# ADVRHumanoids/CentroidalPlanner

Hardware: AMD Instinct MI355X
Metric: NLP eval_g+eval_jac_g throughput (rows/sec) at batch*contacts; HBM GB/s vs peak (higher is better)
Workload: dtype f64; 1 GPU; 4-contact Ground env, batch=1,048,576 (north-star target); contacts=4, environment=ground, batch_per_gpu=1048576, batch_total=1048576, outputs=g + jac (IFOPT CSR values), per-shard residual norms, parallelism=instance-sharded x1, launch=hip-graph, 10 steps per replay

## Files before the change

centroidalplanner_amd/csrc/cpl_kernels.hip:

```cpp
#include <hip/hip_runtime.h>

#include <cmath>
#include <cstdlib>
#include <cstring>
#include <map>
#include <mutex>
#include <string>
#include <tuple>
#include <vector>

#include "cpl_accept.hpp"
#include "cpl_kkt_block.hpp"
#include "cpl_kkt_wave.hpp"
#include "cpl_layout.hpp"
#include "cpl_wave.hpp"
#include "cpl_status.hpp"

namespace cpl {

constexpr int TILE = 64;
constexpr int CHUNK = 16;
constexpr int SROW = CHUNK + 2;

struct KParams {
// ... 723 lines not shown
        __builtin_nontemporal_store(v.y, &d2[e].y);
      } else {
        d2[e] = s2[e];
      }
    }
    if ((count & 1) && tid == 0) dst[count - 1] = src[count - 1];
  } else {
    for (int e = tid; e < count; e += WG) dst[e] = src[e];
  }
}

template <int WG, bool NT>
__device__ __forceinline__ void copy_out_rows(double* __restrict__ dst, const long long* __restrict__ rowb,
                                              const double* __restrict__ src, int rec, int valid, int tid) {
  const int r2 = rec >> 1;
  const int wave = tid >> 6, lane = tid & 63;
  const double2* s2 = reinterpret_cast<const double2*>(src);
  for (int r = wave; r < valid; r += WG / 64) {
    const int b = __builtin_amdgcn_readfirstlane((int)rowb[r]);
    double2* d = reinterpret_cast<double2*>(dst + (int64_t)b * rec);
    const double2* sr = s2 + r * r2;
    for (int q = lane; q < r2; q += 64) {
      const double2 v = sr[q];
      if (NT) {
        __builtin_nontemporal_store(v.x, &d[q].x);
        __builtin_nontemporal_store(v.y, &d[q].y);
      } else {
        d[q] = v;
      }
    }
  }
}

template <int ENVK>
__device__ __forceinline__ void contact_item(const KParams& K, const double* __restrict__ xr, int kind, int k,
                                             double* __restrict__ Gr, double* __restrict__ Jr) {
  const int i = s_ct.map_order[k];
  const double* q = xr + 3 + 9 * i;
  const double F0 = q[0], F1 = q[1], F2 = q[2];
  const double p0 = q[3], p1 = q[4], p2 = q[5];
  const double n0 = q[6], n1 = q[7], n2 = q[8];
  const bool wg = K.want_g, wj = K.want_j;
  double* gk = Gr + 6 + (K.has_env ? 6 : 2) * k;
  double* jk = Jr + K.jbase + K.cstride * k;
  if (ENVK != CPL_ENV_NONE) {
    double gv[4], ej[3], nj[3][3];
    if (ENVK == CPL_ENV_GROUND || (ENVK == CPL_ENV_MIXED && kind == CPL_ENV_GROUND)) {
      gv[0] = p2 - K.ground_z;
      gv[1] = n0 - 0.0; gv[2] = n1 - 0.0; gv[3] = n2 - 1.0;
      ej[0] = 0.0; ej[1] = 0.0; ej[2] = 1.0;
#pragma unroll
      for (int r = 0; r < 3; ++r)
#pragma unroll
        for (int c = 0; c < 3; ++c) nj[r][c] = 0.0;
    } else {
      SQContact s;
      superquadric_contact(K, p0, p1, p2, wj, s);
      gv[0] = s.val;
      gv[1] = n0 - s.en[0]; gv[2] = n1 - s.en[1]; gv[3] = n2 - s.en[2];
#pragma unroll
      for (int r = 0; r < 3; ++r) {
        ej[r] = s.ej[r];
#pragma unroll
        for (int c = 0; c < 3; ++c) nj[r][c] = wj ? s.nj[r][c] : 0.0;
      }
    }
    if (wg) { gk[0] = gv[0]; gk[1] = gv[1]; gk[2] = gv[2]; gk[3] = gv[3]; }
    if (wj && K.fold == FOLD_NONE) {
      jk[0] = ej[0]; jk[1] = ej[1]; jk[2] = ej[2];
#pragma unroll
      for (int r = 0; r < 3; ++r) {
        jk[3 + 4 * r] = nj[r][0]; jk[4 + 4 * r] = nj[r][1]; jk[5 + 4 * r] = nj[r][2]; jk[6 + 4 * r] = 1.0;
      }
      jk += 15;
    } else if (wj && K.fold == FOLD_COMMON) {
      jk[0] = ej[0]; jk[1] = ej[1]; jk[2] = ej[2];
#pragma unroll
      for (int r = 0; r < 3; ++r) { jk[3 + 3 * r] = nj[r][0]; jk[4 + 3 * r] = nj[r][1]; jk[5 + 3 * r] = nj[r][2]; }
      jk += 12;
    }
    gk += 4;
  }
  const double mu = K.mu;
  const double t1 = dot3(F0, F1, F2, n0, n1, n2);
  if (wg) {
    const double nF = dot3(n0, n1, n2, F0, F1, F2);
    const double u0 = F0 - nF * n0, u1 = F1 - nF * n1, u2 = F2 - nF * n2;
    gk[0] = -t1 + s_ct.F_thr[i];
    gk[1] = sqrt((u0 * u0 + u1 * u1) + u2 * u2) - mu * t1;
  }
  if (wj) {
    const double t2 = F0 - n0 * t1;
    const double t3 = F1 - n1 * t1;
    const double t4 = F2 - n2 * t1;
    const double t5 = F0 * n0;
    const double t6 = F1 * n1;
    const double t7 = F2 * n2;
    const double s = sqrt(t2 * t2 + t3 * t3 + t4 * t4);
    jk[0] = -n0; jk[1] = -n1; jk[2] = -n2;
    jk[3] = -F0; jk[4] = -F1; jk[5] = -F2;
    jk[6] = (t2 * (n0 * n0 - 1.0) * 2.0 + n0 * n1 * t3 * 2.0 + n0 * n2 * t4 * 2.0) * 1.0 / s * (-1.0 / 2.0) - mu * n0;
    jk[7] = (t3 * (n1 * n1 - 1.0) * 2.0 + n0 * n1 * t2 * 2.0 + n1 * n2 * t4 * 2.0) * 1.0 / s * (-1.0 / 2.0) - mu * n1;
    jk[8] = (t4 * (n2 * n2 - 1.0) * 2.0 + n0 * n2 * t2 * 2.0 + n1 * n2 * t3 * 2.0) * 1.0 / s * (-1.0 / 2.0) - mu * n2;
    jk[9] = (t2 * (t6 + t7 + t5 * 2.0) * 2.0 + F0 * n1 * t3 * 2.0 + F0 * n2 * t4 * 2.0) * 1.0 / s * (-1.0 / 2.0) - mu * F0;
    jk[10] = (t3 * (t5 + t7 + t6 * 2.0) * 2.0 + F1 * n0 * t2 * 2.0 + F1 * n2 * t4 * 2.0) * 1.0 / s * (-1.0 / 2.0) - mu * F1;
    jk[11] = (t4 * (t5 + t6 + t7 * 2.0) * 2.0 + F2 * n0 * t2 * 2.0 + F2 * n1 * t3 * 2.0) * 1.0 / s * (-1.0 / 2.0) - mu * F2;
  }
}

struct TemplateSrc {
  __device__ __forceinline__ double wrench(const KParams& K, int t) const { return K.wrench[t]; }
  __device__ __forceinline__ double com_ref(const KParams& K, int a) const { return K.com_ref[a]; }
  __device__ __forceinline__ double p_ref(const KParams& K, int i, int a) const { return K.p_ref[i][a]; }
  __device__ __forceinline__ double F_ref(const KParams& K, int i, int a) const { return K.F_ref[i][a]; }
};
struct InstSrc {
  const double* w;
  const double* c;
  const double* p;
  const double* F;
  __device__ __forceinline__ double wrench(const KParams&, int t) const { return w[t]; }
  __device__ __forceinline__ double com_ref(const KParams&, int a) const { return c[a]; }
  __device__ __forceinline__ double p_ref(const KParams&, int i, int a) const { return p[3 * i + a]; }
  __device__ __forceinline__ double F_ref(const KParams&, int i, int a) const { return F[3 * i + a]; }
};

template <class SRC = TemplateSrc>
__device__ __forceinline__ void statics_values_item(const KParams& K, const double* __restrict__ xr, double m_i,
                                                    double* __restrict__ Gr, double* __restrict__ Jr,
                                                    bool with_j = true, double* __restrict__ com6 = nullptr,
                                                    bool pairs_j = false, const SRC& src = SRC()) {
  const int N = K.N;
  if (pairs_j && K.want_j) {
    com6 = Jr + (K.fold == FOLD_NONE ? 3 * N : 0);
  }
  const bool pairs = com6 != nullptr, vals = K.want_g != 0;
  if (pairs || vals) {
    const double c0 = xr[0], c1 = xr[1], c2 = xr[2];
    double v0 = 0.0, v1 = 0.0, v2 = 0.0, v3 = 0.0, v4 = 0.0, v5 = 0.0;
    double a[6] = {0.0, 0.0, 0.0, 0.0, 0.0, 0.0};
    for (int k0 = 0; k0 < N; k0 += 4) {
      double q[4][6];
#pragma unroll
      for (int u = 0; u < 4; ++u) {
        const double* qq = xr + 3 + 9 * s_ct.map_order[k0 + u < N ? k0 + u : k0];
#pragma unroll
        for (int e = 0; e < 6; ++e) q[u][e] = qq[e];
      }
#pragma unroll
      for (int u = 0; u < 4; ++u) {
        if (k0 + u >= N) break;
        const double F0 = q[u][0], F1 = q[u][1], F2 = q[u][2];
        if (pairs) {
          a[0] -= -(-1.0) * F2; a[1] -= -(1.0) * F1;
          a[2] -= -(1.0) * F2;  a[3] -= -(-1.0) * F0;
          a[4] -= -(-1.0) * F1; a[5] -= -(1.0) * F0;
        }
        if (vals) {
          const double d0 = q[u][3] - c0, d1 = q[u][4] - c1, d2 = q[u][5] - c2;
          v0 += F0; v1 += F1; v2 += F2;
          v3 += d1 * F2 - d2 * F1;
          v4 += d2 * F0 - d0 * F2;
          v5 += d0 * F1 - d1 * F0;
        }
      }
    }
    if (pairs) {
      if (pairs_j) {
#pragma unroll
        for (int t = 0; t < 6; ++t) com6[(t >> 1) * (2 + 4 * N) + (t & 1)] = a[t];
      } else {
#pragma unroll
        for (int t = 0; t < 6; ++t) com6[t] = a[t];
      }
    }
    if (vals) {
      v0 -= src.wrench(K, 0); v1 -= src.wrench(K, 1); v2 -= src.wrench(K, 2);
      v3 -= src.wrench(K, 3); v4 -= src.wrench(K, 4); v5 -= src.wrench(K, 5);
      v0 += m_i * K.gravity[0]; v1 += m_i * K.gravity[1]; v2 += m_i * K.gravity[2];
      Gr[0] = v0; Gr[1] = v1; Gr[2] = v2; Gr[3] = v3; Gr[4] = v4; Gr[5] = v5;
    }
  }
  if (with_j && K.want_j && K.fold == FOLD_NONE)
    for (int e = 0; e < 3 * N; ++e) Jr[e] = 1.0;
}

__device__ __forceinline__ void statics_rows_coop(const KParams& K, const double* __restrict__ xr,
                                                  const double* __restrict__ com6, double* __restrict__ Jr, int tid,
                                                  int nthreads) {
  const int N = K.N;
  const int RL = 2 + 4 * N;
  const int I3 = K.fold == FOLD_NONE ? 3 * N : 0;
  const int SJ = I3 + 3 * RL;
  for (int e = tid; e < SJ; e += nthreads) {
    double v = 1.0;
    if (e >= I3) {
      int w = e - I3;
      const int q = w >= 2 * RL ? 2 : (w >= RL ? 1 : 0);
      w -= q * RL;
      const int e1 = q == 2 ? 1 : 2;
      const int e2 = q == 0 ? 1 : 0;
      const double s1 = q == 1 ? 1.0 : -1.0;
      const double s2 = q == 1 ? -1.0 : 1.0;
      if (w < 2) {
        v = com6[2 * q + w];
      } else {
        const int i = (w - 2) >> 2, c = (w - 2) & 3;
        const double* F = xr + 3 + 9 * i;
        const double* p = F + 3;
        v = c == 0 ? s1 * (p[e1] - xr[e1]) : c == 1 ? s2 * (p[e2] - xr[e2]) : c == 2 ? -s1 * F[e1] : -s2 * F[e2];
      }
    }
    Jr[e] = v;
  }
}

__device__ __forceinline__ void statics_row_item(const KParams& K, const double* __restrict__ xr, int q,
                                                 double* __restrict__ Jr) {
  const int N = K.N;
  const int e1 = q == 2 ? 1 : 2;
  const int e2 = q == 0 ? 1 : 0;
  const double s1 = q == 1 ? 1.0 : -1.0;
  const double s2 = q == 1 ? -1.0 : 1.0;
  const double ce1 = xr[e1], ce2 = xr[e2];
  double a1 = 0.0, a2 = 0.0;
  for (int k = 0; k < N; ++k) {
    const double* F = xr + 3 + 9 * s_ct.map_order[k];
    a1 -= -s1 * F[e1];
    a2 -= -s2 * F[e2];
  }
  double* row = Jr + (K.fold == FOLD_NONE ? 3 * N : 0) + q * (2 + 4 * N);
  row[0] = a1;
  row[1] = a2;
  for (int i = 0; i < N; ++i) {
    const double* F = xr + 3 + 9 * i;
    const double* p = F + 3;
    row[2 + 4 * i] = s1 * (p[e1] - ce1);
    row[3 + 4 * i] = s2 * (p[e2] - ce2);
    row[4 + 4 * i] = -s1 * F[e1];
    row[5 + 4 * i] = -s2 * F[e2];
  }
}

template <class SRC = TemplateSrc>
__device__ __forceinline__ double cost_value(const KParams& K, const double* __restrict__ xr, const SRC& src = SRC()) {
  const int N = K.N;
  double value = 0;
  for (int k = 0; k < N; ++k) {
    const int i = s_ct.map_order[k];
    const double* q = xr + 3 + 9 * i;
    const double e0 = q[3] - src.p_ref(K, i, 0), e1 = q[4] - src.p_ref(K, i, 1), e2 = q[5] - src.p_ref(K, i, 2);
    const double h0 = q[0] - src.F_ref(K, i, 0), h1 = q[1] - src.F_ref(K, i, 1), h2 = q[2] - src.F_ref(K, i, 2);
    value += 0.5 * K.W_p[i] * ((e0 * e0 + e1 * e1) + e2 * e2) + 0.5 * K.W_F[i] * ((h0 * h0 + h1 * h1) + h2 * h2);
  }
  const double r0 = xr[0] - src.com_ref(K, 0), r1 = xr[1] - src.com_ref(K, 1), r2 = xr[2] - src.com_ref(K, 2);
  value += 0.5 * K.W_com * ((r0 * r0 + r1 * r1) + r2 * r2);
  return value;
}

template <class SRC = TemplateSrc>
__device__ __forceinline__ void cost_item(const KParams& K, const double* __restrict__ xr, double* __restrict__ f,
                                          double* __restrict__ Dr, const double* __restrict__ fscale = nullptr,
                                          const SRC& src = SRC()) {
  const int N = K.N;
// ... 626 lines not shown
    }
    if (K.want_lgrad) {
      for (int e = tid; e < valid * n; e += CT) {
        const int r = e / n, j = e - r * n;
        if (K.lg_active && !K.lg_active[(b0 + r) / K.y_repeat]) continue;
        const double* jr = Jt + r * nnz;
        const double* yb = K.ly + ((b0 + r) / K.y_repeat) * m;
        double s = Dt[r * n + j];
        for (int q = s_colp[j]; q < s_colp[j + 1]; ++q) {
          double v = jr[s_csck[q]];
          v = v == v ? v : 0.0;
          s += v * yb[s_cscr[q]];
        }
        grad_out[(b0 + r) * n + j] = s;
      }
    } else if (K.soa) {
      if (K.want_g) copy_out_soa<CT, NT>(g_out + b0, batch, Gt, m, valid, tid);
      if (K.want_j) copy_out_soa<CT, NT>(jac_out + b0, batch, Jt, nnz, valid, tid);
      if (K.want_grad) copy_out_soa<CT, NT>(grad_out + b0, batch, Dt, n, valid, tid);
    } else {
      if (K.want_g) copy_out_ct<CT, NT>(g_out + b0 * m, Gt, valid * m, tid);
      if (K.want_j) copy_out_ct<CT, NT>(jac_out + b0 * nnz, Jt, valid * nnz, tid);
      if (K.want_grad) copy_out_ct<CT, NT>(grad_out + b0 * n, Dt, valid * n, tid);
    }
    if (K.want_norms) acc.add_tile(Gt, valid * m, tid, CT, m);
    lds_barrier();
    cur ^= 1;
  }
  }
  if (K.want_norms) partial_norms(acc, norms_ws + NORM_HDR);
}
using PipeKernT = void (*)(const KParams, int64_t, const double*, const double*, const uint8_t*, double*, double*,
                           double*, double*, double*);


constexpr int ENT_PC = 15;
enum { EPC_D = 0, EPC_ROW1 = 3, EPC_CONEG = 9, EPC_ENVG = 11, EPC_NORMG = 12 };
constexpr unsigned OP_X = 0u << 28, OP_S = 1u << 28, OP_C = 2u << 28, OP_NEG = 1u << 31;

template <int ENVK>
__device__ __forceinline__ unsigned entry_op_g(int q, int S0) {
  constexpr int CR = ENVK == CPL_ENV_NONE ? 2 : 6;
  if (q < 6) return OP_S | (unsigned)q;
  const int u = q - 6, k = u / CR, w = u - k * CR;
  const unsigned ci = (unsigned)(S0 + ENT_PC * s_ct.map_order[k]);
  if (ENVK == CPL_ENV_NONE) return OP_S | (ci + EPC_CONEG + w);
  if (w == 0) return OP_S | (ci + EPC_ENVG);
  if (w < 4) return OP_S | (ci + EPC_NORMG + (w - 1));
  return OP_S | (ci + EPC_CONEG + (w - 4));
}
template <int ENVK>
__device__ __forceinline__ unsigned entry_op_j(int q, int N, int S0) {
  constexpr int CJ = ENVK == CPL_ENV_NONE ? 12 : 27;
  const int RL = 2 + 4 * N, JC = 3 * N + 3 * RL;
  if (q < 3 * N) return OP_C | 1u;
  if (q < JC) {
    int w = q - 3 * N;
    const int qq = w >= 2 * RL ? 2 : (w >= RL ? 1 : 0);
    w -= qq * RL;
    if (w < 2) return OP_S | (unsigned)(6 + 2 * qq + w);
    const int e1 = qq == 2 ? 1 : 2, e2 = qq == 0 ? 1 : 0;
    const bool s1neg = qq != 1, s2neg = qq == 1;
    const int i = (w - 2) >> 2, c = (w - 2) & 3;
    const unsigned ci = (unsigned)(S0 + ENT_PC * i);
    switch (c) {
      case 0: return OP_S | (ci + EPC_D + e1) | (s1neg ? OP_NEG : 0u);
// ... 737 lines not shown
    K.C[a] = C; K.R[a] = R; K.P[a] = P;
    if (sq) {
      K.EJ[a] = cache.EJ[a]; K.Ka[a] = cache.Ka[a]; K.Kb[a] = cache.Kb[a];
      K.Rm2[a] = cache.Rm2[a]; K.Rp2[a] = cache.Rp2[a];
    }
    K.Psq[a] = P * P;
    K.Pm1[a] = P - 1.0;
    K.P2[a] = P * 2.0;
    K.P2m2[a] = P * 2.0 - 2.0;
    K.P2m3[a] = P * 2.0 - 3.0;
  }
  K.sq_ladder = 1;
  for (int a = 0; a < 3; ++a) {
    const double P = d->sq_P[a];
    if (!(P >= 2.0 && P <= 64.0 && P == std::floor(P))) K.sq_ladder = 0;
  }
  for (int i = 0; i < CPL_MAX_CONTACTS; ++i) {
    K.F_thr[i] = d->F_thr[i];
    K.W_p[i] = d->W_p[i];
    K.W_F[i] = d->W_F[i];
    for (int j = 0; j < 3; ++j) { K.p_ref[i][j] = d->p_ref[i][j]; K.F_ref[i][j] = d->F_ref[i][j]; }
  }
  K.W_com = d->W_com;
  for (int j = 0; j < 3; ++j) K.com_ref[j] = d->com_ref[j];
  K.fold = FOLD_NONE;
  K.jbase = D.statics_nnz;
  K.cstride = D.contact_nnz;
  K.soa = 0;
}

static size_t eval_lds_bytes(int n) { return sizeof(double) * (size_t)(TILE * n + 2 * TILE * SROW); }

enum { VAR_AUTO = 0, VAR_ROWSTAGE = 1, VAR_PIPE = 2, VAR_TILE = 3, VAR_TILE_JD = 4, VAR_ENTRY = 5, VAR_SPLIT = 6,
       VAR_SPLIT_JD = 7 };
static int g_variant = VAR_AUTO;
static size_t g_lds_budget = 0;
static int g_wg = 256;
static int g_nt = 1;

static size_t tile_budget() { return g_lds_budget ? g_lds_budget : 48 * 1024; }
static size_t pipe_budget() { return g_lds_budget ? g_lds_budget : 48 * 1024; }
static bool use_rowstage() { return g_variant == VAR_ROWSTAGE; }
static bool use_pipe(const KParams& K) {
  if (!K.x_aligned16) return false;
  if (g_variant == VAR_PIPE) return true;
  return g_variant == VAR_AUTO && (K.env_kind == CPL_ENV_NONE || K.env_kind == CPL_ENV_GROUND);
}

static int32_t plan_tile(KParams& K, bool g, bool j, bool f, bool grad, int t_max = 64, bool size_without_j = false) {
  const size_t budget = tile_budget();
  K.want_g = g; K.want_j = j; K.want_f = f; K.want_grad = grad;
  const bool sq = K.env_kind == CPL_ENV_SUPERQUADRIC || K.env_kind == CPL_ENV_MIXED;
  K.LR = K.N * SQ_L + 1;
  const size_t per = sizeof(double) * (size_t)(K.n + (g ? K.m : 0) + (j && !K.jdirect ? K.nnz : 0) +
                                               (grad ? K.n : 0) + (sq ? K.LR : 0) + (j && K.jdirect ? 6 : 0));
  const size_t per_t = size_without_j ? per - sizeof(double) * (size_t)(j && !K.jdirect ? K.nnz : 0) : per;
  const size_t fixed = sizeof(double) * 72 + sizeof(CTab);
  int T = 64, logT = 6;
  while (T > t_max) { T >>= 1; --logT; }
  while (T > 2 && (size_t)T * per_t + fixed > budget) { T >>= 1; --logT; }
  if ((size_t)T * per + fixed > 160 * 1024) return fail(CPL_ERR_UNSUPPORTED, "problem too large for one LDS tile");
  K.T = T; K.logT = logT;
  K.cost_seg = (f || grad) ? K.N + 4 : -1;
  K.S = K.N + 4 + ((f || grad) ? 1 : 0);
  K.offG = T * K.n;
  K.offJ = K.offG + (g ? T * K.m : 0);
  K.offD = K.offJ + (j && !K.jdirect ? T * K.nnz : 0);
  K.offL = K.offD + (grad ? T * K.n : 0);
  K.offA = K.offL + (sq ? T * K.LR : 0);
  K.offI = K.offA + (j && K.jdirect ? 6 * T : 0);
  K.offI = (K.offI + 1) & ~1;
  K.offRB = K.offI + 72;
  return CPL_OK;
}

static int32_t plan_pipe(KParams& K, bool g, bool j, bool f, bool grad, size_t extra_fixed = 0) {
  K.want_g = g; K.want_j = j; K.want_f = f; K.want_grad = grad;
  const bool sq = K.env_kind == CPL_ENV_SUPERQUADRIC || K.env_kind == CPL_ENV_MIXED;
// ... 140 lines not shown
  if (c.norms && (st = norm_workspace(C, c.stream, nparts, &ws))) return st;
  if ((st = side_stream(C, c.stream))) return st;
  hipError_t e = hipEventRecord(C.fork, c.stream);
  if (e == hipSuccess) e = hipStreamWaitEvent(C.side, C.fork, 0);
  if (e != hipSuccess) return hip_fail(e, "mixed split fork");
  hipLaunchKernelGGL(tk, dim3(grid_s), dim3(256), lds_s, c.stream, Ks, batch, c.x, c.mass, c.env_tag, kl.idx_sq,
                     kl.counts + 1, c.g, c.jac, c.f, c.grad, ws ? ws + 2 * (size_t)grid_g : nullptr);
  hipLaunchKernelGGL(ek, dim3(grid_g), dim3(256), lds_g, C.side, Kg, batch, c.x, c.mass, kl.idx_gr, kl.counts, c.g,
                     c.jac, c.f, c.grad, ws);
  e = hipGetLastError();
  if (e != hipSuccess) return hip_fail(e, "mixed split launch");
  e = hipEventRecord(C.join, C.side);
  if (e == hipSuccess) e = hipStreamWaitEvent(c.stream, C.join, 0);
  if (e != hipSuccess) return hip_fail(e, "mixed split join");
  return launched(c, "mixed split launch", nparts, ws);
}

static int32_t launch_entry(const EvalCall& c, KParams& K, StreamCtx* C) {
  int32_t st = plan_entry(K, c.g != nullptr, c.jac != nullptr, c.f != nullptr, c.grad != nullptr);
  if (st) return st;
  const size_t lds = sizeof(double) * (size_t)K.offI;
  static const EntryKernT table[2][2] = {
      {cpl_eval_entry_kernel<CPL_ENV_NONE, false>, cpl_eval_entry_kernel<CPL_ENV_NONE, true>},
      {cpl_eval_entry_kernel<CPL_ENV_GROUND, false>, cpl_eval_entry_kernel<CPL_ENV_GROUND, true>}};
  const EntryKernT kern = table[K.env_kind == CPL_ENV_GROUND ? 1 : 0][g_nt ? 1 : 0];
  const unsigned grid = persistent_grid((c.batch + K.T - 1) / K.T, reinterpret_cast<const void*>(kern), lds);
  double* ws = nullptr;
  if (c.norms && (st = norm_workspace(*C, c.stream, grid, &ws))) return st;
  hipLaunchKernelGGL(kern, dim3(grid), dim3(256), lds, c.stream, K, c.batch, c.x, c.mass, nullptr, nullptr, c.g, c.jac,
                     c.f, c.grad, ws);
  return launched(c, "cpl_eval_entry_kernel launch", grid, ws);
}

static int32_t launch_pipe(const EvalCall& c, KParams& K, StreamCtx* C) {
  const LGradArgs* lg = c.lg;
  const int csc_doubles = lg ? (K.n + 1 + 2 * K.nnz + 1) / 2 : 0;
  int32_t st = lg ? plan_pipe(K, false, true, false, true, sizeof(double) * (size_t)csc_doubles)
                  : plan_pipe(K, c.g != nullptr, c.jac != nullptr, c.f != nullptr, c.grad != nullptr);
  if (st) return st;
  K.offC = K.offI + 72;
  if (lg) {
    K.want_lgrad = 1;
    K.y_repeat = lg->y_repeat;
    K.col_ptr = lg->col_ptr;
    K.csc_k = lg->csc_k;
    K.csc_row = lg->csc_row;
    K.ly = lg->y;
    K.lg_active = lg->active;
  }
  const size_t lds = sizeof(double) * (size_t)(K.offC + csc_doubles);
  static const PipeKernT table[4][2] = {
      {cpl_eval_pipe_kernel<CPL_ENV_NONE, 3, false>, cpl_eval_pipe_kernel<CPL_ENV_NONE, 3, true>},
      {cpl_eval_pipe_kernel<CPL_ENV_GROUND, 3, false>, cpl_eval_pipe_kernel<CPL_ENV_GROUND, 3, true>},
      {cpl_eval_pipe_kernel<CPL_ENV_SUPERQUADRIC, 3, false>, cpl_eval_pipe_kernel<CPL_ENV_SUPERQUADRIC, 3, true>},
      {cpl_eval_pipe_kernel<CPL_ENV_MIXED, 3, false>, cpl_eval_pipe_kernel<CPL_ENV_MIXED, 3, true>}};
  static const PipeKernT table_sc[2][2] = {
      {cpl_eval_pipe_kernel<CPL_ENV_NONE, 3, false, true>, cpl_eval_pipe_kernel<CPL_ENV_NONE, 3, true, true>},
      {cpl_eval_pipe_kernel<CPL_ENV_GROUND, 3, false, true>, cpl_eval_pipe_kernel<CPL_ENV_GROUND, 3, true, true>}};
  if (c.sc && K.env_kind != CPL_ENV_NONE && K.env_kind != CPL_ENV_GROUND) return CPL_ERR_UNSUPPORTED;
  if (c.sc) {
    K.sc_df = c.sc->df;
    K.sc_dc = c.sc->dc;
    K.sc_row = c.sc->row;
  }
  const PipeKernT kern =
      c.sc ? table_sc[K.env_kind == CPL_ENV_GROUND ? 1 : 0][g_nt ? 1 : 0] : table[K.env_kind][g_nt ? 1 : 0];
  const unsigned grid = persistent_grid((c.batch + K.T - 1) / K.T, reinterpret_cast<const void*>(kern), lds);
  double* ws = nullptr;
  if (c.norms && (st = norm_workspace(*C, c.stream, grid, &ws))) return st;
  hipLaunchKernelGGL(kern, dim3(grid), dim3(256), lds, c.stream, K, c.batch, c.x, c.mass, c.env_tag, c.g, c.jac, c.f,
                     c.grad, ws);
  return launched(c, "cpl_eval_pipe_kernel launch", grid, ws);
}

static int32_t launch_rowstage(const EvalCall& c, const KParams& K) {
  const size_t lds = eval_lds_bytes(K.n);
  if (lds > 160 * 1024) return fail(CPL_ERR_UNSUPPORTED, "problem too large for one LDS tile");
  const unsigned grid = (unsigned)((c.batch + TILE - 1) / TILE);
  hipLaunchKernelGGL(cpl_eval_kernel, dim3(grid), dim3(TILE), lds, c.stream, K, c.batch, c.x, c.mass, c.env_tag, c.g,
                     c.jac, c.f, c.grad);
  if (int32_t st = launched(c, "cpl_eval_kernel launch")) return st;
  return c.norms && c.finish ? cpl_residual_norms(c.d, c.batch, c.g, c.norms, c.stream) : CPL_OK;
}

static int32_t launch_tile(const EvalCall& c, KParams& K, StreamCtx* C) {
  const bool jd = g_variant == VAR_TILE_JD || (g_variant == VAR_AUTO && K.env_kind == CPL_ENV_MIXED);
  const int wg = g_wg;
  K.jdirect = (jd && c.jac && !K.soa && wg == 256) ? 1 : 0;
  int32_t st = plan_tile(K, c.g != nullptr, c.jac != nullptr, c.f != nullptr, c.grad != nullptr, 64, jd && c.jac);
  if (st) return st;
  const size_t lds = sizeof(double) * (size_t)(K.offRB + K.T);
  const unsigned grid = (unsigned)((c.batch + K.T - 1) / K.T);
  const size_t nparts = (size_t)grid * (wg / 64);
  double* ws = nullptr;
  if (c.norms && (st = norm_workspace(*C, c.stream, nparts, &ws))) return st;
#define CPL_TILE_KERNELS(E) \
  {cpl_eval_tile_kernel<E, 128, false, false>, cpl_eval_tile_kernel<E, 128, true, false>,        \
   cpl_eval_tile_kernel<E, 256, false, false>, cpl_eval_tile_kernel<E, 256, true, false>,        \
   cpl_eval_tile_kernel<E, 256, false, true>, cpl_eval_tile_kernel<E, 256, true, true>}
// ... 11 lines not shown
  int32_t st = validate_desc(d);
  if (st) return st;
  if (c.flags & ~(CPL_EVAL_JAC_FOLDED | CPL_EVAL_SOA)) return fail(CPL_ERR_INVALID_ARGUMENT, "unknown eval flags");
  if (c.batch < 0) return fail(CPL_ERR_INVALID_ARGUMENT, "negative batch");
  if (c.batch == 0) {
    if (c.norms) {
      hipError_t e = hipMemsetAsync(c.norms, 0, 2 * sizeof(double), c.stream);
      if (e != hipSuccess) return hip_fail(e, "hipMemsetAsync norms");
    }
    return CPL_OK;
  }
  if (c.norms && !c.g) return fail(CPL_ERR_INVALID_ARGUMENT, "residual norms need the g output");
  if (!c.x) return fail(CPL_ERR_INVALID_ARGUMENT, "x is required");
  if (d->env_kind == CPL_ENV_MIXED && !c.env_tag)
    return fail(CPL_ERR_INVALID_ARGUMENT, "mixed environment batch needs a per-instance env tag array");
  if ((c.batch + 7) / 8 > 0x7fffffffLL) return fail(CPL_ERR_INVALID_ARGUMENT, "batch too large");
  if (!c.g && !c.jac && !c.f && !c.grad) return CPL_OK;
  KParams K;
  fill_params(d, K, c.x);
  K.gate = c.gate;
  if (c.flags & CPL_EVAL_JAC_FOLDED) {
    K.fold = fold_level(d->env_kind);
    K.nnz = folded_nnz(K.N, d->env_kind);
    K.jbase = 6 + 12 * K.N;
    K.cstride = folded_contact_nnz(d->env_kind);
  }
  K.soa = (c.flags & CPL_EVAL_SOA) ? 1 : 0;
  K.want_norms = c.norms != nullptr;
  K.y_repeat = 1;
  const bool split = !c.lg && use_split(K, c.flags, c.batch), entry = !c.lg && use_entry(K, c.flags);
  if (c.sc && (c.lg || c.norms || K.soa || !use_pipe(K) || split || entry)) return CPL_ERR_UNSUPPORTED;
  if (c.lg && !use_pipe(K))
    return fail(CPL_ERR_UNSUPPORTED, "fused Lagrangian gradient: pipelined (Ground / no environment) path only");
  StreamCtx* C = nullptr;
  if ((split || c.norms) && (st = stream_ctx(c.stream, &C))) return st;
  if (split && (g_variant != VAR_AUTO || split_ready(*C, c.stream, c.batch))) return launch_split(c, K, *C);
  if (entry) return launch_entry(c, K, C);
  if (use_pipe(K)) return launch_pipe(c, K, C);
  if (use_rowstage() && c.flags == 0) return launch_rowstage(c, K);
  return launch_tile(c, K, C);
}

struct InstPtrs {
  const double *wrench, *com_ref, *p_ref, *F_ref;
  bool any() const { return wrench || com_ref || p_ref || F_ref; }
};

template <bool NT>
__global__ __launch_bounds__(256) void cpl_inst_overlay_kernel(const KParams K, int64_t batch,
                                                               const double* __restrict__ x,
                                                               const double* __restrict__ mass, const InstPtrs I,
                                                               double* __restrict__ g_out, double* __restrict__ f_out,
                                                               double* __restrict__ grad_out) {
  extern __shared__ __align__(16) double smem[];
  if (K.gate && *K.gate == 0) return;
  const int tid = threadIdx.x;
  const int T = K.T, n = K.n, m = K.m, N = K.N;
  const int64_t b0 = (int64_t)blockIdx.x * T;
  if (b0 >= batch) return;
  const int valid = (int)((batch - b0) < T ? (batch - b0) : T);
  double* X = smem;
  double* Dt = X + T * n;
  double* G6 = Dt + T * n;
  double* Fv = G6 + T * 6;
  double* Wl = Fv + T;
  double* Cl = Wl + T * 6;
// ... 479 lines not shown
                               void* stream) {
  int32_t st = validate_desc(d);
  if (st) return st;
  if (d->env_kind != CPL_ENV_GROUND && d->env_kind != CPL_ENV_NONE)
    return fail(CPL_ERR_UNSUPPORTED, "cpl_lagrangian_hessian: Ground / no-environment problems only");
  return launch_hessian("cpl_lagrangian_hessian", d, batch, d_x, d_y, nullptr, d_active, d_free_idx, nf, d_H, stream);
}

int32_t cpl_lagrangian_hessian_ex(const cpl_problem_desc* d, int64_t batch, const double* d_x, const double* d_y,
                                  const uint8_t* d_env_tag, const uint8_t* d_active, const int32_t* d_free_idx,
                                  int32_t nf, double* d_H, void* stream) {
  int32_t st = validate_desc(d);
  if (st) return st;
  return launch_hessian("cpl_lagrangian_hessian_ex", d, batch, d_x, d_y, d_env_tag, d_active, d_free_idx, nf, d_H,
                        stream);
}

int32_t cpl_eval_batch_ex(const cpl_problem_desc* d, int64_t batch, const double* d_x, const double* d_mass,
                          const uint8_t* d_env_tag, double* d_g, double* d_jac, double* d_f, double* d_grad,
                          double* d_norms, int32_t flags, void* stream) {
  return launch_eval(EvalCall{d, batch, d_x, d_mass, d_env_tag, d_g, d_jac, d_f, d_grad, d_norms, (hipStream_t)stream, flags});
}

int32_t cpl_eval_batch_norms(const cpl_problem_desc* d, int64_t batch, const double* d_x, const double* d_mass,
                             const uint8_t* d_env_tag, double* d_g, double* d_jac, double* d_f, double* d_grad,
                             double* d_norms, void* stream) {
  if (!d_norms) return fail(CPL_ERR_INVALID_ARGUMENT, "d_norms is required");
  return launch_eval(EvalCall{d, batch, d_x, d_mass, d_env_tag, d_g, d_jac, d_f, d_grad, d_norms, (hipStream_t)stream});
}

int32_t cpl_set_tuning(int32_t kernel_variant, int32_t tile_lds_kb, int32_t wg_threads, int32_t nt_stores,
                       int32_t reserved ) {
  if (reserved != 0) return fail(CPL_ERR_INVALID_ARGUMENT, "the fifth tuning argument is reserved and must be 0");
  if (kernel_variant < VAR_AUTO || kernel_variant > VAR_SPLIT_JD) return fail(CPL_ERR_INVALID_ARGUMENT, "unknown kernel variant");
  if (tile_lds_kb != 0 && (tile_lds_kb < 8 || tile_lds_kb > 160))
    return fail(CPL_ERR_INVALID_ARGUMENT, "LDS budget out of [8, 160] KiB");
  if (wg_threads != 128 && wg_threads != 256) return fail(CPL_ERR_INVALID_ARGUMENT, "workgroup size must be 128 or 256");
  g_variant = kernel_variant;
  g_lds_budget = (size_t)tile_lds_kb * 1024;
  g_wg = wg_threads;
  g_nt = nt_stores ? 1 : 0;
  return CPL_OK;
}

int32_t cpl_residual_norms(const cpl_problem_desc* d, int64_t batch, const double* d_g, double* d_out, void* stream) {
  int32_t st = validate_desc(d);
  if (st) return st;
  if (batch < 0 || !d_out || (batch > 0 && !d_g)) return fail(CPL_ERR_INVALID_ARGUMENT, "bad residual arguments");
  hipStream_t s = (hipStream_t)stream;
  StreamCtx* C = nullptr;
  if ((st = stream_ctx(s, &C))) return st;
  if ((st = ctx_reserve(s, C->rn, RN_GRID, sizeof(double) * 2 * RN_GRID, "residual norms: the per-stream workspace")))
    return st;
  double* ws = static_cast<double*>(C->rn.ptr);
  const Dims D = dims_of(d->n_contacts, d->env_kind);
  const int64_t total = batch * D.m;
  int64_t blocks = (total + RN_BLOCK - 1) / RN_BLOCK;
  if (blocks < 1) blocks = 1;
  if (blocks > RN_GRID) blocks = RN_GRID;
  hipLaunchKernelGGL(cpl_residual_partial, dim3((unsigned)blocks), dim3(RN_BLOCK), 0, s, total, D.m, D.contact_rows,
                     d_g, ws);
  hipError_t e = hipGetLastError();
  if (e != hipSuccess) return hip_fail(e, "cpl_residual_partial launch");
  launch_residual_final((int)blocks, ws, d_out, s);
  e = hipGetLastError();
  if (e != hipSuccess) return hip_fail(e, "cpl_residual_final launch");
  return CPL_OK;
// ... 42 lines not shown
```

Baseline: 78.70 billion rows/s.

## Add fixed-shape pipelined kernel specialised for 4 contacts with hoisted constant Jacobian entries

Adds a compile-time specialised pipelined kernel for N=4 contacts (no environment or Ground). It writes the constant Jacobian entries (ones and ground zeros) into shared memory once per block instead of every tile, and splits the cone Jacobian work across waves. It also uses register-staged copy-out with compile-time trip counts. The default auto path picks this kernel when the layout matches the generic pipe kernel's offsets, at the cost of more code paths and a risk of layout mismatch.

```diff
diff --git a/centroidalplanner_amd/csrc/cpl_kernels.hip b/centroidalplanner_amd/csrc/cpl_kernels.hip
--- a/centroidalplanner_amd/csrc/cpl_kernels.hip
+++ b/centroidalplanner_amd/csrc/cpl_kernels.hip
@@ -779,6 +779,53 @@
   }
 }
 
+struct ConeArgs { double F0, F1, F2, n0, n1, n2; };
+struct ConeTerms { double t2, t3, t4, t5, t6, t7, s; };
+
+__device__ __forceinline__ void ground_values(double p2, double n0, double n1, double n2, double ground_z,
+                                              double* __restrict__ gv) {
+  gv[0] = p2 - ground_z;
+  gv[1] = n0 - 0.0; gv[2] = n1 - 0.0; gv[3] = n2 - 1.0;
+}
+
+__device__ __forceinline__ void cone_values(const ConeArgs& a, double t1, double F_thr, double mu,
+                                            double* __restrict__ gk) {
+  const double F0 = a.F0, F1 = a.F1, F2 = a.F2, n0 = a.n0, n1 = a.n1, n2 = a.n2;
+  const double nF = dot3(n0, n1, n2, F0, F1, F2);
+  const double u0 = F0 - nF * n0, u1 = F1 - nF * n1, u2 = F2 - nF * n2;
+  gk[0] = -t1 + F_thr;
+  gk[1] = sqrt((u0 * u0 + u1 * u1) + u2 * u2) - mu * t1;
+}
+
+__device__ __forceinline__ ConeTerms cone_terms(const ConeArgs& a, double t1) {
+  ConeTerms t;
+  t.t2 = a.F0 - a.n0 * t1;
+  t.t3 = a.F1 - a.n1 * t1;
+  t.t4 = a.F2 - a.n2 * t1;
+  t.t5 = a.F0 * a.n0;
+  t.t6 = a.F1 * a.n1;
+  t.t7 = a.F2 * a.n2;
+  t.s = sqrt(t.t2 * t.t2 + t.t3 * t.t3 + t.t4 * t.t4);
+  return t;
+}
+__device__ __forceinline__ void cone_row0(const ConeArgs& a, double* __restrict__ jk) {
+  jk[0] = -a.n0; jk[1] = -a.n1; jk[2] = -a.n2;
+  jk[3] = -a.F0; jk[4] = -a.F1; jk[5] = -a.F2;
+}
+template <int E>
+__device__ __forceinline__ double cone_row1(const ConeArgs& a, const ConeTerms& t, double mu) {
+  const double F0 = a.F0, F1 = a.F1, F2 = a.F2, n0 = a.n0, n1 = a.n1, n2 = a.n2;
+  const double t2 = t.t2, t3 = t.t3, t4 = t.t4, t5 = t.t5, t6 = t.t6, t7 = t.t7, s = t.s;
+  switch (E) {
+    case 0: return (t2 * (n0 * n0 - 1.0) * 2.0 + n0 * n1 * t3 * 2.0 + n0 * n2 * t4 * 2.0) * 1.0 / s * (-1.0 / 2.0) - mu * n0;
+    case 1: return (t3 * (n1 * n1 - 1.0) * 2.0 + n0 * n1 * t2 * 2.0 + n1 * n2 * t4 * 2.0) * 1.0 / s * (-1.0 / 2.0) - mu * n1;
+    case 2: return (t4 * (n2 * n2 - 1.0) * 2.0 + n0 * n2 * t2 * 2.0 + n1 * n2 * t3 * 2.0) * 1.0 / s * (-1.0 / 2.0) - mu * n2;
+    case 3: return (t2 * (t6 + t7 + t5 * 2.0) * 2.0 + F0 * n1 * t3 * 2.0 + F0 * n2 * t4 * 2.0) * 1.0 / s * (-1.0 / 2.0) - mu * F0;
+    case 4: return (t3 * (t5 + t7 + t6 * 2.0) * 2.0 + F1 * n0 * t2 * 2.0 + F1 * n2 * t4 * 2.0) * 1.0 / s * (-1.0 / 2.0) - mu * F1;
+    default: return (t4 * (t5 + t6 + t7 * 2.0) * 2.0 + F2 * n0 * t2 * 2.0 + F2 * n1 * t3 * 2.0) * 1.0 / s * (-1.0 / 2.0) - mu * F2;
+  }
+}
+
 template <int ENVK>
 __device__ __forceinline__ void contact_item(const KParams& K, const double* __restrict__ xr, int kind, int k,
                                              double* __restrict__ Gr, double* __restrict__ Jr) {
@@ -793,8 +840,7 @@
   if (ENVK != CPL_ENV_NONE) {
     double gv[4], ej[3], nj[3][3];
     if (ENVK == CPL_ENV_GROUND || (ENVK == CPL_ENV_MIXED && kind == CPL_ENV_GROUND)) {
-      gv[0] = p2 - K.ground_z;
-      gv[1] = n0 - 0.0; gv[2] = n1 - 0.0; gv[3] = n2 - 1.0;
+      ground_values(p2, n0, n1, n2, K.ground_z, gv);
       ej[0] = 0.0; ej[1] = 0.0; ej[2] = 1.0;
 #pragma unroll
       for (int r = 0; r < 3; ++r)
@@ -829,31 +875,39 @@
     gk += 4;
   }
   const double mu = K.mu;
+  const ConeArgs a{F0, F1, F2, n0, n1, n2};
   const double t1 = dot3(F0, F1, F2, n0, n1, n2);
-  if (wg) {
-    const double nF = dot3(n0, n1, n2, F0, F1, F2);
-    const double u0 = F0 - nF * n0, u1 = F1 - nF * n1, u2 = F2 - nF * n2;
-    gk[0] = -t1 + s_ct.F_thr[i];
-    gk[1] = sqrt((u0 * u0 + u1 * u1) + u2 * u2) - mu * t1;
-  }
+  if (wg) cone_values(a, t1, s_ct.F_thr[i], mu, gk);
   if (wj) {
-    const double t2 = F0 - n0 * t1;
-    const double t3 = F1 - n1 * t1;
-    const double t4 = F2 - n2 * t1;
-    const double t5 = F0 * n0;
-    const double t6 = F1 * n1;
-    const double t7 = F2 * n2;
-    const double s = sqrt(t2 * t2 + t3 * t3 + t4 * t4);
-    jk[0] = -n0; jk[1] = -n1; jk[2] = -n2;
-    jk[3] = -F0; jk[4] = -F1; jk[5] = -F2;
-    jk[6] = (t2 * (n0 * n0 - 1.0) * 2.0 + n0 * n1 * t3 * 2.0 + n0 * n2 * t4 * 2.0) * 1.0 / s * (-1.0 / 2.0) - mu * n0;
-    jk[7] = (t3 * (n1 * n1 - 1.0) * 2.0 + n0 * n1 * t2 * 2.0 + n1 * n2 * t4 * 2.0) * 1.0 / s * (-1.0 / 2.0) - mu * n1;
-    jk[8] = (t4 * (n2 * n2 - 1.0) * 2.0 + n0 * n2 * t2 * 2.0 + n1 * n2 * t3 * 2.0) * 1.0 / s * (-1.0 / 2.0) - mu * n2;
-    jk[9] = (t2 * (t6 + t7 + t5 * 2.0) * 2.0 + F0 * n1 * t3 * 2.0 + F0 * n2 * t4 * 2.0) * 1.0 / s * (-1.0 / 2.0) - mu * F0;
-    jk[10] = (t3 * (t5 + t7 + t6 * 2.0) * 2.0 + F1 * n0 * t2 * 2.0 + F1 * n2 * t4 * 2.0) * 1.0 / s * (-1.0 / 2.0) - mu * F1;
-    jk[11] = (t4 * (t5 + t6 + t7 * 2.0) * 2.0 + F2 * n0 * t2 * 2.0 + F2 * n1 * t3 * 2.0) * 1.0 / s * (-1.0 / 2.0) - mu * F2;
-  }
-}
+    const ConeTerms t = cone_terms(a, t1);
+    cone_row0(a, jk);
+    jk[6] = cone_row1<0>(a, t, mu);
+    jk[7] = cone_row1<1>(a, t, mu);
+    jk[8] = cone_row1<2>(a, t, mu);
+    jk[9] = cone_row1<3>(a, t, mu);
+    jk[10] = cone_row1<4>(a, t, mu);
+    jk[11] = cone_row1<5>(a, t, mu);
+  }
+}
+
+struct LaunchShape {
+  static constexpr bool writes_constants = true;
+  __device__ __forceinline__ int N(const KParams& K) const { return K.N; }
+  __device__ __forceinline__ bool want_g(const KParams& K) const { return K.want_g != 0; }
+  __device__ __forceinline__ bool want_j(const KParams& K) const { return K.want_j != 0; }
+  __device__ __forceinline__ int fold(const KParams& K) const { return K.fold; }
+  __device__ __forceinline__ int order(int k) const { return s_ct.map_order[k]; }
+};
+template <int NF>
+struct FixedShape {
+  static constexpr bool writes_constants = false;
+  int mo[NF];
+  __device__ __forceinline__ constexpr int N(const KParams&) const { return NF; }
+  __device__ __forceinline__ constexpr bool want_g(const KParams&) const { return true; }
+  __device__ __forceinline__ constexpr bool want_j(const KParams&) const { return true; }
+  __device__ __forceinline__ constexpr int fold(const KParams&) const { return FOLD_NONE; }
+  __device__ __forceinline__ int order(int k) const { return mo[k]; }
+};
 
 struct TemplateSrc {
   __device__ __forceinline__ double wrench(const KParams& K, int t) const { return K.wrench[t]; }
@@ -872,16 +926,17 @@
   __device__ __forceinline__ double F_ref(const KParams&, int i, int a) const { return F[3 * i + a]; }
 };
 
-template <class SRC = TemplateSrc>
+template <class SRC = TemplateSrc, class SH = LaunchShape>
 __device__ __forceinline__ void statics_values_item(const KParams& K, const double* __restrict__ xr, double m_i,
                                                     double* __restrict__ Gr, double* __restrict__ Jr,
                                                     bool with_j = true, double* __restrict__ com6 = nullptr,
-                                                    bool pairs_j = false, const SRC& src = SRC()) {
-  const int N = K.N;
-  if (pairs_j && K.want_j) {
-    com6 = Jr + (K.fold == FOLD_NONE ? 3 * N : 0);
-  }
-  const bool pairs = com6 != nullptr, vals = K.want_g != 0;
+                                                    bool pairs_j = false, const SRC& src = SRC(),
+                                                    const SH& sh = SH()) {
+  const int N = sh.N(K);
+  if (pairs_j && sh.want_j(K)) {
+    com6 = Jr + (sh.fold(K) == FOLD_NONE ? 3 * N : 0);
+  }
+  const bool pairs = com6 != nullptr, vals = sh.want_g(K);
   if (pairs || vals) {
     const double c0 = xr[0], c1 = xr[1], c2 = xr[2];
     double v0 = 0.0, v1 = 0.0, v2 = 0.0, v3 = 0.0, v4 = 0.0, v5 = 0.0;
@@ -890,7 +945,7 @@
       double q[4][6];
 #pragma unroll
       for (int u = 0; u < 4; ++u) {
-        const double* qq = xr + 3 + 9 * s_ct.map_order[k0 + u < N ? k0 + u : k0];
+        const double* qq = xr + 3 + 9 * sh.order(k0 + u < N ? k0 + u : k0);
 #pragma unroll
         for (int e = 0; e < 6; ++e) q[u][e] = qq[e];
       }
@@ -928,7 +983,7 @@
       Gr[0] = v0; Gr[1] = v1; Gr[2] = v2; Gr[3] = v3; Gr[4] = v4; Gr[5] = v5;
     }
   }
-  if (with_j && K.want_j && K.fold == FOLD_NONE)
+  if (SH::writes_constants && with_j && sh.want_j(K) && sh.fold(K) == FOLD_NONE)
     for (int e = 0; e < 3 * N; ++e) Jr[e] = 1.0;
 }
 
@@ -962,9 +1017,10 @@
   }
 }
 
+template <class SH = LaunchShape>
 __device__ __forceinline__ void statics_row_item(const KParams& K, const double* __restrict__ xr, int q,
-                                                 double* __restrict__ Jr) {
-  const int N = K.N;
+                                                 double* __restrict__ Jr, const SH& sh = SH()) {
+  const int N = sh.N(K);
   const int e1 = q == 2 ? 1 : 2;
   const int e2 = q == 0 ? 1 : 0;
   const double s1 = q == 1 ? 1.0 : -1.0;
@@ -972,11 +1028,11 @@
   const double ce1 = xr[e1], ce2 = xr[e2];
   double a1 = 0.0, a2 = 0.0;
   for (int k = 0; k < N; ++k) {
-    const double* F = xr + 3 + 9 * s_ct.map_order[k];
+    const double* F = xr + 3 + 9 * sh.order(k);
     a1 -= -s1 * F[e1];
     a2 -= -s2 * F[e2];
   }
-  double* row = Jr + (K.fold == FOLD_NONE ? 3 * N : 0) + q * (2 + 4 * N);
+  double* row = Jr + (sh.fold(K) == FOLD_NONE ? 3 * N : 0) + q * (2 + 4 * N);
   row[0] = a1;
   row[1] = a2;
   for (int i = 0; i < N; ++i) {
@@ -1669,6 +1725,217 @@
 }
 using PipeKernT = void (*)(const KParams, int64_t, const double*, const double*, const uint8_t*, double*, double*,
                            double*, double*, double*);
+
+template <int ENVK, int N>
+struct PipeFixed {
+  static_assert(ENVK == CPL_ENV_NONE || ENVK == CPL_ENV_GROUND, "fixed-shape kernel: no environment or Ground");
+  static constexpr bool ENV = ENVK != CPL_ENV_NONE;
+  static constexpr int NCW = 3, CT = 64 * NCW;
+  static constexpr int n = 3 + 9 * N, CR = ENV ? 6 : 2, CJ = ENV ? 27 : 12;
+  static constexpr int m = 6 + CR * N, SJ = 6 + 15 * N, nnz = SJ + CJ * N;
+  static constexpr int up2(int v) { return (v + 1) & ~1; }
+  static constexpr int tile_log() {
+    int T = 64, logT = 6;
+    while (T > 8 && sizeof(double) * (size_t)T * (2 * n + 3 + m + nnz) + sizeof(double) * 80 + sizeof(CTab) > 48 * 1024) {
+      T >>= 1;
+      --logT;
+    }
+    return logT;
+  }
+  static constexpr int LOGT = tile_log(), T = 1 << LOGT;
+  static constexpr int offX1 = up2(T * n), offMB = offX1 + up2(T * n), offTB = offMB + 2 * T, offG = offTB + T,
+                       offJ = offG + T * m, offI = up2(offJ + T * nnz);
+  static_assert(m % 2 == 0 && nnz % 2 == 0, "records of whole 16-byte pairs");
+};
+
+template <int CT, bool NT, bool FULL, int PG, int PJ>
+__device__ __forceinline__ void copy_out_fixed(double* __restrict__ g_dst, double* __restrict__ j_dst,
+                                               const double* __restrict__ Gt, const double* __restrict__ Jt, int pg,
+                                               int pj, int tid) {
+  constexpr int TG = (PG + CT - 1) / CT, TJ = (PJ + CT - 1) / CT;
+  const double2* sg = reinterpret_cast<const double2*>(Gt);
+  const double2* sj = reinterpret_cast<const double2*>(Jt);
+  double2* dg = reinterpret_cast<double2*>(g_dst);
+  double2* dj = reinterpret_cast<double2*>(j_dst);
+  double2 vg[TG], vj[TJ];
+#pragma unroll
+  for (int i = 0; i < TG; ++i) vg[i] = sg[(i + 1) * CT <= PG || tid + i * CT < PG ? tid + i * CT : tid];
+#pragma unroll
+  for (int i = 0; i < TJ; ++i) vj[i] = sj[(i + 1) * CT <= PJ || tid + i * CT < PJ ? tid + i * CT : tid];
+  auto put = [](double2* d, const double2 v) {
+    if (NT) {
+      __builtin_nontemporal_store(v.x, &d->x);
+      __builtin_nontemporal_store(v.y, &d->y);
+    } else {
+      *d = v;
+    }
+  };
+#pragma unroll
+  for (int i = 0; i < TG; ++i) {
+    const int e = tid + i * CT;
+    if (FULL ? ((i + 1) * CT <= PG || e < PG) : e < pg) put(dg + e, vg[i]);
+  }
+#pragma unroll
+  for (int i = 0; i < TJ; ++i) {
+    const int e = tid + i * CT;
+    if (FULL ? ((i + 1) * CT <= PJ || e < PJ) : e < pj) put(dj + e, vj[i]);
+  }
+}
+
+template <int ENVK, int N, bool NT>
+__global__ __launch_bounds__(256) void cpl_eval_pipe_fixed_kernel(const KParams K, int64_t batch,
+                                                                  const double* __restrict__ x,
+                                                                  const double* __restrict__ mass,
+                                                                  const uint8_t* __restrict__ ,
+                                                                  double* __restrict__ g_out,
+                                                                  double* __restrict__ jac_out,
+                                                                  double* __restrict__ ,
+                                                                  double* __restrict__ ,
+                                                                  double* __restrict__ norms_ws) {
+  using FS = PipeFixed<ENVK, N>;
+  constexpr int NCW = FS::NCW, CT = FS::CT, T = FS::T, LOGT = FS::LOGT, n = FS::n, m = FS::m, nnz = FS::nnz;
+  constexpr int SJ = FS::SJ, CJ = FS::CJ, CR = FS::CR;
+  constexpr bool ENV = FS::ENV;
+  constexpr int CTRIPS = (N * T + 63) / 64, STRIPS = (4 * T + 63) / 64;
+  extern __shared__ __align__(16) double smem[];
+  load_ctab(K);
+  __syncthreads();
+  const int tid = threadIdx.x;
+  const int lane = tid & 63, wave = tid >> 6;
+  const bool loader = wave == NCW;
+  const int64_t ntiles = (batch + T - 1) >> LOGT;
+  auto XB = [&](int bi) { return smem + (bi ? FS::offX1 : 0); };
+  auto MB = [&](int bi) { return smem + FS::offMB + (bi ? T : 0); };
+  double* Gt = smem + FS::offG;
+  double* Jt = smem + FS::offJ;
+
+  int64_t t = blockIdx.x;
+  if (t >= ntiles) return;
+  double mass_def = K.mass_default;
+  asm volatile("" : "+v"(mass_def));
+  NormAcc acc;
+  acc.init(tid, CT, m);
+
+  if (loader) {
+    double st_mass = 0.0, st_tail = 0.0;
+    auto stage = [&](int64_t tt, int bi) {
+      const int64_t b0s = tt << LOGT;
+      const int vs = (int)((batch - b0s) < T ? (batch - b0s) : T);
+      const int count = vs * n;
+      dma_tile(XB(bi), x + b0s * n, count, lane);
+      if ((count & 1) && lane == 0) st_tail = x[b0s * n + count - 1];
+      if (lane < vs) st_mass = mass ? mass[b0s + lane] : mass_def;
+    };
+    auto finish_stage = [&](int64_t tt, int bi) {
+      asm volatile("s_waitcnt vmcnt(0)" ::: "memory");
+      const int64_t b0s = tt << LOGT;
+      const int vs = (int)((batch - b0s) < T ? (batch - b0s) : T);
+      const int count = vs * n;
+      if ((count & 1) && lane == 0) XB(bi)[count - 1] = st_tail;
+      if (lane < vs) MB(bi)[lane] = st_mass;
+    };
+    __builtin_amdgcn_s_setprio(3);
+    stage(t, 0);
+    finish_stage(t, 0);
+    lds_barrier();
+    int cur = 0;
+    for (; t < ntiles; t += gridDim.x) {
+      const int64_t tn = t + gridDim.x;
+      if (tn < ntiles) stage(tn, cur ^ 1);
+      lds_barrier();
+      if (tn < ntiles) finish_stage(tn, cur ^ 1);
+      lds_barrier();
+      cur ^= 1;
+    }
+  } else {
+    FixedShape<N> sh;
+#pragma unroll
+    for (int k = 0; k < N; ++k) sh.mo[k] = __builtin_amdgcn_readfirstlane(s_ct.map_order[k]);
+    int ci[CTRIPS];
+    double fthr[CTRIPS];
+#pragma unroll
+    for (int u = 0; u < CTRIPS; ++u) {
+      const int k = (lane + 64 * u) >> LOGT;
+      ci[u] = s_ct.map_order[k < N ? k : 0];
+      fthr[u] = s_ct.F_thr[ci[u]];
+    }
+    const double mu = K.mu, ground_z = K.ground_z;
+    for (int e = tid; e < T * 3 * N; e += CT) Jt[(e / (3 * N)) * nnz + e % (3 * N)] = 1.0;
+    if (ENV)
+      for (int e = tid; e < T * N * 15; e += CT) {
+        const int r = e / (N * 15), w = e % (N * 15), c = w % 15;
+        Jt[r * nnz + SJ + CJ * (w / 15) + c] = (c == 2 || (c >= 3 && ((c - 3) & 3) == 3)) ? 1.0 : 0.0;
+      }
+    lds_barrier();
+    int cur = 0;
+    for (; t < ntiles; t += gridDim.x) {
+      const int64_t b0 = t << LOGT;
+      const int valid = (int)((batch - b0) < T ? (batch - b0) : T);
+      const double* X = XB(cur);
+      if (wave < 2) {
+#pragma unroll
+        for (int u = 0; u < CTRIPS; ++u) {
+          const int it = lane + 64 * u, r = it & (T - 1), k = it >> LOGT;
+          if (it >= N * T || r >= valid) continue;
+          const double* q = X + r * n + 3 + 9 * ci[u];
+          const ConeArgs a{q[0], q[1], q[2], q[6], q[7], q[8]};
+          const ConeTerms ct = cone_terms(a, dot3(a.F0, a.F1, a.F2, a.n0, a.n1, a.n2));
+          double* jk = Jt + r * nnz + SJ + CJ * k + (ENV ? 15 : 0);
+          if (wave == 0) {
+            jk[6] = cone_row1<0>(a, ct, mu);
+            jk[7] = cone_row1<1>(a, ct, mu);
+            jk[8] = cone_row1<2>(a, ct, mu);
+          } else {
+            jk[9] = cone_row1<3>(a, ct, mu);
+            jk[10] = cone_row1<4>(a, ct, mu);
+            jk[11] = cone_row1<5>(a, ct, mu);
+          }
+        }
+      } else {
+#pragma unroll
+        for (int u = 0; u < CTRIPS; ++u) {
+          const int it = lane + 64 * u, r = it & (T - 1), k = it >> LOGT;
+          if (it >= N * T || r >= valid) continue;
+          const double* q = X + r * n + 3 + 9 * ci[u];
+          const ConeArgs a{q[0], q[1], q[2], q[6], q[7], q[8]};
+          double* gk = Gt + r * m + 6 + CR * k;
+          double* jk = Jt + r * nnz + SJ + CJ * k;
+          if (ENV) {
+            double gv[4];
+            ground_values(q[5], a.n0, a.n1, a.n2, ground_z, gv);
+            gk[0] = gv[0]; gk[1] = gv[1]; gk[2] = gv[2]; gk[3] = gv[3];
+            gk += 4;
+            jk += 15;
+          }
+          cone_values(a, dot3(a.F0, a.F1, a.F2, a.n0, a.n1, a.n2), fthr[u], mu, gk);
+          cone_row0(a, jk);
+        }
+#pragma unroll
+        for (int u = 0; u < STRIPS; ++u) {
+          const int it = lane + 64 * u, r = it & (T - 1), sg = it >> LOGT;
+          if (it >= 4 * T || r >= valid) continue;
+          const double* xr = X + r * n;
+          if (sg == 0)
+            statics_values_item<TemplateSrc, FixedShape<N>>(K, xr, MB(cur)[r], Gt + r * m, Jt + r * nnz, true, nullptr,
+                                                            false, TemplateSrc(), sh);
+          else
+            statics_row_item(K, xr, sg - 1, Jt + r * nnz, sh);
+        }
+      }
+      lds_barrier();
+      if (valid == T)
+        copy_out_fixed<CT, NT, true, T * m / 2, T * nnz / 2>(g_out + b0 * m, jac_out + b0 * nnz, Gt, Jt, T * m / 2,
+                                                            T * nnz / 2, tid);
+      else
+        copy_out_fixed<CT, NT, false, T * m / 2, T * nnz / 2>(g_out + b0 * m, jac_out + b0 * nnz, Gt, Jt,
+                                                             valid * m / 2, (valid * nnz) >> 1, tid);
+      if (K.want_norms) acc.add_tile(Gt, valid * m, tid, CT, m);
+      lds_barrier();
+      cur ^= 1;
+    }
+  }
+  if (K.want_norms) partial_norms(acc, norms_ws + NORM_HDR);
+}
 
 
 constexpr int ENT_PC = 15;
@@ -2472,7 +2739,7 @@
 static size_t eval_lds_bytes(int n) { return sizeof(double) * (size_t)(TILE * n + 2 * TILE * SROW); }
 
 enum { VAR_AUTO = 0, VAR_ROWSTAGE = 1, VAR_PIPE = 2, VAR_TILE = 3, VAR_TILE_JD = 4, VAR_ENTRY = 5, VAR_SPLIT = 6,
-       VAR_SPLIT_JD = 7 };
+       VAR_SPLIT_JD = 7, VAR_UNASSIGNED = 8 , VAR_PIPE_FIXED = 9 };
 static int g_variant = VAR_AUTO;
 static size_t g_lds_budget = 0;
 static int g_wg = 256;
@@ -2483,7 +2750,7 @@
 static bool use_rowstage() { return g_variant == VAR_ROWSTAGE; }
 static bool use_pipe(const KParams& K) {
   if (!K.x_aligned16) return false;
-  if (g_variant == VAR_PIPE) return true;
+  if (g_variant == VAR_PIPE || g_variant == VAR_PIPE_FIXED) return true;
   return g_variant == VAR_AUTO && (K.env_kind == CPL_ENV_NONE || K.env_kind == CPL_ENV_GROUND);
 }
 
@@ -2690,6 +2957,29 @@
   return launched(c, "cpl_eval_entry_kernel launch", grid, ws);
 }
 
+struct PipeFixedEntry {
+  int32_t env_kind, N, T, offG, offJ, offI;
+  PipeKernT kern[2];
+};
+#define CPL_PIPE_FIXED_ONE(E, N) \
+  {E, N, PipeFixed<E, N>::T, PipeFixed<E, N>::offG, PipeFixed<E, N>::offJ, PipeFixed<E, N>::offI, \
+   {cpl_eval_pipe_fixed_kernel<E, N, false>, cpl_eval_pipe_fixed_kernel<E, N, true>}}
+#define CPL_PIPE_FIXED(N) CPL_PIPE_FIXED_ONE(CPL_ENV_NONE, N), CPL_PIPE_FIXED_ONE(CPL_ENV_GROUND, N)
+static const PipeFixedEntry g_pipe_fixed[] = {
+    CPL_PIPE_FIXED(4),
+};
+#undef CPL_PIPE_FIXED
+#undef CPL_PIPE_FIXED_ONE
+
+static PipeKernT pipe_fixed_kernel(const EvalCall& c, const KParams& K) {
+  if (c.flags != 0 || !c.g || !c.jac || c.f || c.grad || c.lg || c.sc || c.gate || !K.x_aligned16) return nullptr;
+  if (((reinterpret_cast<uintptr_t>(c.g) | reinterpret_cast<uintptr_t>(c.jac)) & 15) != 0) return nullptr;
+  for (const PipeFixedEntry& e : g_pipe_fixed)
+    if (e.env_kind == K.env_kind && e.N == K.N)
+      return e.T == K.T && e.offG == K.offG && e.offJ == K.offJ && e.offI == K.offI ? e.kern[g_nt ? 1 : 0] : nullptr;
+  return nullptr;
+}
+
 static int32_t launch_pipe(const EvalCall& c, KParams& K, StreamCtx* C) {
   const LGradArgs* lg = c.lg;
   const int csc_doubles = lg ? (K.n + 1 + 2 * K.nnz + 1) / 2 : 0;
@@ -2721,8 +3011,12 @@
     K.sc_dc = c.sc->dc;
     K.sc_row = c.sc->row;
   }
-  const PipeKernT kern =
-      c.sc ? table_sc[K.env_kind == CPL_ENV_GROUND ? 1 : 0][g_nt ? 1 : 0] : table[K.env_kind][g_nt ? 1 : 0];
+  const PipeKernT fixed = g_variant == VAR_PIPE ? nullptr : pipe_fixed_kernel(c, K);
+  if (g_variant == VAR_PIPE_FIXED && !fixed)
+    return fail(CPL_ERR_UNSUPPORTED, "fixed-shape pipelined kernel: this launch is outside its conditions");
+  const PipeKernT kern = fixed ? fixed
+                         : c.sc ? table_sc[K.env_kind == CPL_ENV_GROUND ? 1 : 0][g_nt ? 1 : 0]
+                                : table[K.env_kind][g_nt ? 1 : 0];
   const unsigned grid = persistent_grid((c.batch + K.T - 1) / K.T, reinterpret_cast<const void*>(kern), lds);
   double* ws = nullptr;
   if (c.norms && (st = norm_workspace(*C, c.stream, grid, &ws))) return st;
@@ -2800,6 +3094,8 @@
   if (c.sc && (c.lg || c.norms || K.soa || !use_pipe(K) || split || entry)) return CPL_ERR_UNSUPPORTED;
   if (c.lg && !use_pipe(K))
     return fail(CPL_ERR_UNSUPPORTED, "fused Lagrangian gradient: pipelined (Ground / no environment) path only");
+  if (g_variant == VAR_PIPE_FIXED && !use_pipe(K))
+    return fail(CPL_ERR_UNSUPPORTED, "fixed-shape pipelined kernel: x is not 16-byte aligned");
   StreamCtx* C = nullptr;
   if ((split || c.norms) && (st = stream_ctx(c.stream, &C))) return st;
   if (split && (g_variant != VAR_AUTO || split_ready(*C, c.stream, c.batch))) return launch_split(c, K, *C);
@@ -3345,7 +3641,7 @@
 int32_t cpl_set_tuning(int32_t kernel_variant, int32_t tile_lds_kb, int32_t wg_threads, int32_t nt_stores,
                        int32_t reserved ) {
   if (reserved != 0) return fail(CPL_ERR_INVALID_ARGUMENT, "the fifth tuning argument is reserved and must be 0");
-  if (kernel_variant < VAR_AUTO || kernel_variant > VAR_SPLIT_JD) return fail(CPL_ERR_INVALID_ARGUMENT, "unknown kernel variant");
+  if (kernel_variant < VAR_AUTO || kernel_variant > VAR_PIPE_FIXED || kernel_variant == VAR_UNASSIGNED) return fail(CPL_ERR_INVALID_ARGUMENT, "unknown kernel variant");
   if (tile_lds_kb != 0 && (tile_lds_kb < 8 || tile_lds_kb > 160))
     return fail(CPL_ERR_INVALID_ARGUMENT, "LDS budget out of [8, 160] KiB");
   if (wg_threads != 128 && wg_threads != 256) return fail(CPL_ERR_INVALID_ARGUMENT, "workgroup size must be 128 or 256");
```

Measured after the change: 80.44 billion rows/s, median of 6. +2.2%, better.
